# alexklwong/calibrated-backprojection-network

Measured on AMD Instinct MI355X. Metric: depth-completion frames/sec at 352x1216, higher is better.
Workload: dtype f32; 1 GPU; KITTI 352x1216, batch 32/GPU, fp32, full KBNet forward in HIP, random xavier weights; frames_per_gpu=32, global_batch=32, height=352, width=1216, n_ranks_seen=1, collective_backend=nccl, gathered_frames=32, launch=HIP graph replay, 2 concurrent sub-batch branch(es)

## Files before the change

### calibrated-backprojection-network_amd/csrc/abi.hip

```cpp
#include <stdlib.h>
#include <string.h>

#include "kbn_common.h"

namespace kbn {

KnobValue g_knobs[KNOB_COUNT];

static const char* const kKnobNames[KNOB_COUNT] = {
    "KBN_DEBUG", "KBN_FORCE_MW", "KBN_FORCE_TWB", "KBN_EPI_LDS", "KBN_NO_WINO",
    "KBN_NO_UP2X9", "KBN_NO_UP2X3", "KBN_WINO_RT",
    "KBN_NO_KB_PAIR", "KBN_NO_KB_DEPTH_FUSION", "KBN_PAIR_CAND", "KBN_S2D_DEBUG", "KBN_AUTOTUNE",
    "KBN_NO_HEAD_FUSION", "KBN_NO_SPLIT", "KBN_NO_OVERLAP", "KBN_NO_PAIR", "KBN_NO_PAIR_MID", "KBN_NO_PAIR_ENC",
    "KBN_NO_PAIR_TAIL", "KBN_NO_DEPTH_FRONT_FUSION", "KBN_FP16_ONE_TERM", "KBN_DEPTH_FRONT_FUSION", "KBN_NO_FRONT_NEXT"};

void tune_reload_env();

static void load_knobs() {
    for (int k = 0; k < KNOB_COUNT; ++k) {
        const char* v = getenv(kKnobNames[k]);
        g_knobs[k].set = (v && *v) ? 1 : 0;
        int val = 0;
        if (v && *v) {
            char* end = nullptr;
            const long parsed = strtol(v, &end, 10);
            val = (end == v) ? 1 : (int)parsed;
        }
        g_knobs[k].value = val;
    }
}

namespace {
struct KnobInit {
    KnobInit() { load_knobs(); }
} g_knob_init;
}

int device_cu_count() {
    static std::atomic<int> cache[256];
    int dev = 0;
    if (hipGetDevice(&dev) != hipSuccess) return -1;
    std::atomic<int>& slot = cache[dev & 255];
    int v = slot.load(std::memory_order_relaxed);
    if (v > 0) return v;
    if (hipDeviceGetAttribute(&v, hipDeviceAttributeMultiprocessorCount, dev) != hipSuccess || v < 1) return -1;
    slot.store(v, std::memory_order_relaxed);
    return v;
}

}

extern "C" {

int kbn_version(void) { return KBN_ABI_VERSION; }

const char* kbn_status_string(int status) {
    switch (status) {
        case KBN_OK: return "ok";
        case KBN_ERR_INVALID_ARGUMENT: return "invalid argument";
        case KBN_ERR_UNSUPPORTED: return "configuration outside the kernel limits";
        case KBN_ERR_WORKSPACE: return "buffer too small";
        case KBN_ERR_LAUNCH: return "HIP launch error";
        default: return "unknown status";
    }
}

int kbn_knob(const char* name) {
    if (!name) return 0;
    for (int k = 0; k < kbn::KNOB_COUNT; ++k)
        if (!strcmp(name, kbn::kKnobNames[k])) return kbn::g_knobs[k].value;
    return 0;
}

void kbn_reload_env(void) {
    kbn::load_knobs();
    kbn::tune_reload_env();
}

}
```

### calibrated-backprojection-network_amd/csrc/kbn_common.h

```cpp
#pragma once

#include <hip/hip_runtime.h>
#include <stdint.h>

#include <atomic>
#include <type_traits>

#include "../../include/kbnet_hip.h"

#define KBN_CHECK_LAUNCH()                                   \
    do {                                                     \
        hipError_t e__ = hipGetLastError();                  \
        if (e__ != hipSuccess) return KBN_ERR_LAUNCH;        \
    } while (0)

namespace kbn {

typedef float f32x4 __attribute__((ext_vector_type(4)));
typedef float f32x2 __attribute__((ext_vector_type(2)));

__host__ __device__ inline int ceil_div(int a, int b) { return (a + b - 1) / b; }
__host__ __device__ inline int round_up(int a, int b) { return ceil_div(a, b) * b; }

__device__ __forceinline__ float leaky_relu(float v, float slope) { return v > 0.f ? v : v * slope; }
__device__ __forceinline__ float fin_abs(float v) { const float a = fabsf(v); return a < __builtin_inff() ? a : 0.f; }

__device__ __forceinline__ unsigned wave_max_bits(float m) {
#define KBN_DPP_MAX(ctrl) m = fmaxf(m, __int_as_float(__builtin_amdgcn_update_dpp(0, __float_as_int(m), ctrl, 0xf, 0xf, true)))
    KBN_DPP_MAX(0xB1);
    KBN_DPP_MAX(0x4E);
    KBN_DPP_MAX(0x141);
    KBN_DPP_MAX(0x140);
#undef KBN_DPP_MAX
    const int v = __float_as_int(m);
    const unsigned a = (unsigned)__builtin_amdgcn_readlane(v, 0), b = (unsigned)__builtin_amdgcn_readlane(v, 16);
    const unsigned c = (unsigned)__builtin_amdgcn_readlane(v, 32), d = (unsigned)__builtin_amdgcn_readlane(v, 48);
    const unsigned ab = a > b ? a : b, cd = c > d ? c : d;
    return ab > cd ? ab : cd;
}
__device__ __forceinline__ float quad_sum(float x) {
    x += __int_as_float(__builtin_amdgcn_update_dpp(0, __float_as_int(x), 0xB1, 0xf, 0xf, true));
    x += __int_as_float(__builtin_amdgcn_update_dpp(0, __float_as_int(x), 0x4E, 0xf, 0xf, true));
    return x;
}
__device__ __forceinline__ void absmax_commit(unsigned* slot, float m) {
    const unsigned b = wave_max_bits(m);
    if ((threadIdx.x & 63) == 0) {
        if (b > __hip_atomic_load(slot, __ATOMIC_RELAXED, __HIP_MEMORY_SCOPE_AGENT)) atomicMax(slot, b);
    }
}
int absmax_frames_launch(const float* x, long long batch_stride, int n, long long per_frame, unsigned* slots, hipStream_t stream);

struct DeviceOnce {
    std::atomic<unsigned long long> done[4] = {};
};
inline int set_max_dynamic_lds(DeviceOnce& once, const void* kernel, int bytes) {
    int dev = 0;
    if (hipGetDevice(&dev) != hipSuccess) return KBN_ERR_LAUNCH;
    const unsigned long long bit = 1ull << (dev & 63);
    std::atomic<unsigned long long>& word = once.done[(dev >> 6) & 3];
    if (word.load(std::memory_order_relaxed) & bit) return KBN_OK;
    if (hipFuncSetAttribute(kernel, hipFuncAttributeMaxDynamicSharedMemorySize, bytes) != hipSuccess)
        return KBN_ERR_LAUNCH;
    word.fetch_or(bit, std::memory_order_relaxed);
    return KBN_OK;
}
template <auto K>
inline DeviceOnce lds_once;
template <auto K, int MAX_LDS, class... Args>
int launch_lds(unsigned blocks, unsigned threads, size_t lds, hipStream_t stream, const Args&... args) {
    if (int rc = set_max_dynamic_lds(lds_once<K>, reinterpret_cast<const void*>(K), MAX_LDS)) return rc;
    hipLaunchKernelGGL(K, dim3(blocks), dim3(threads), lds, stream, args...);
    return KBN_OK;
}
template <class F>
int flag_dispatch(F&& f) { return f(); }
template <class F, class... Flags>
int flag_dispatch(F&& f, bool flag, Flags... rest) {
    auto bind = [&](auto c) { return flag_dispatch([&](auto... more) { return f(c, more...); }, rest...); };
    return flag ? bind(std::true_type{}) : bind(std::false_type{});
}
int device_cu_count();

enum Knob {
    KNOB_DEBUG, KNOB_FORCE_MW, KNOB_FORCE_TWB, KNOB_EPI_LDS, KNOB_NO_WINO,
    KNOB_NO_UP2X9, KNOB_NO_UP2X3, KNOB_WINO_RT,
    KNOB_NO_KB_PAIR, KNOB_NO_KB_DEPTH_FUSION, KNOB_PAIR_CAND, KNOB_S2D_DEBUG, KNOB_AUTOTUNE,
    KNOB_NO_HEAD_FUSION, KNOB_NO_SPLIT,
    KNOB_NO_OVERLAP, KNOB_NO_PAIR, KNOB_NO_PAIR_MID, KNOB_NO_PAIR_ENC, KNOB_NO_PAIR_TAIL, KNOB_NO_DEPTH_FRONT_FUSION,
    KNOB_FP16_ONE_TERM, KNOB_DEPTH_FRONT_FUSION, KNOB_NO_FRONT_NEXT, KNOB_COUNT
};
struct KnobValue { int set, value; };
extern KnobValue g_knobs[KNOB_COUNT];
inline int knob(Knob k) { return g_knobs[k].value; }
inline bool knob_set(Knob k) { return g_knobs[k].set != 0; }

__device__ __forceinline__ int xcd_remap(int bid, int nblocks) {
    const int NX = 8;
    int xcd = bid % NX, idx = bid / NX;
    int q = nblocks / NX, r = nblocks % NX;
    int start = (xcd < r) ? xcd * (q + 1) : r * (q + 1) + (xcd - r) * q;
    return start + idx;
}

__device__ __forceinline__ int nearest_src_index(int dst, int in_size, int out_size) {
    if (in_size == out_size) return dst;
    if (out_size == 2 * in_size) return dst >> 1;
    float scale = (float)in_size / (float)out_size;
    int s = (int)floorf((float)dst * scale);
    return s < in_size - 1 ? s : in_size - 1;
}

int conv2d_launch(const kbn_conv_src* srcs, int n_src, const float* packed_weight, float* out,
                  long long out_batch_stride, int n, int out_channels, int kernel_size, int stride,
                  int in_height, int in_width, int resize, int apply_activation, float negative_slope,
                  unsigned* out_absmax, hipStream_t stream);

}
```

### calibrated-backprojection-network_amd/csrc/s2d.hip

```cpp
#include <math.h>

#include <initializer_list>

#include "kbn_common.h"
#include "s2d_pools.h"

namespace kbn {

constexpr int S2D_TW = 64, S2D_TH = 16, S2D_THREADS = 256;
constexpr int S2D_FW = S2D_TW + 2, S2D_FH = S2D_TH + 2;
constexpr int S2D_NQ = (S2D_FW + 3) / 4;
constexpr int S2D_FWP = S2D_NQ * 4;
constexpr int S2D_GS = 6;
constexpr int S2D_MAXPOOL = 8, S2D_MAXF = 8, S2D_MAXCONV = 4, S2D_MAXIN = 2, S2D_MAXR = 15;
constexpr int S2D_MAXCH = S2D_MAXF + S2D_MAXIN;
constexpr int S2D_W3 = S2D_MAXCH * 9 * 8, S2D_W1 = S2D_MAXCONV * 8 * 8;
constexpr int S2D_WFLOATS = S2D_W3 + S2D_W1;
static_assert(S2D_FH % S2D_GS == 0 && S2D_TH % 4 == 0, "tile geometry");

struct S2DParams {
    const float* x;
    long long x_bstride;
    float* out;
    float* pyramid;
    const float* wpool[S2D_MAXCONV];
    const float* wconv;
    int N, H, W, inC;
    int nmin, npool;
    int ksize[S2D_MAXPOOL];
    int nconv, nf, R, Rmin, Rmax;
    int tilesX, tilesY, nblocks;
    int dbg;
    float slope;
};

__host__ __device__ constexpr int s2d_zw(int R) { return S2D_FW + 2 * R; }
__host__ __device__ constexpr int s2d_zh(int R) { return S2D_FH + 2 * R; }
__host__ __device__ constexpr int s2d_vp(int R) { return (S2D_FWP + 2 * R + 3) / 4 * 4; }

struct DynamicPools {
    static constexpr bool is_static = false;
    static constexpr int RMAXZ = S2D_MAXR;
    __device__ static int R(const S2DParams& p) { return p.R; }
};

__device__ __forceinline__ float s2d_lrelu(float v, float slope) {
    float t = v * slope, o;
    asm("v_max_f32 %0, %1, %2" : "=v"(o) : "v"(v), "v"(t));
    return o;
}

__device__ __forceinline__ f32x4 mfma4(float a, float b, f32x4 c) {
    return __builtin_amdgcn_mfma_f32_4x4x1f32(a, b, c, 0, 0, 0);
}

template <typename CFG>
__global__ __launch_bounds__(S2D_THREADS, 2) void s2d_kernel(const S2DParams p) {
    extern __shared__ __attribute__((aligned(16))) float smem[];
    const int R = CFG::R(p);
    const int ZW = s2d_zw(R), ZH = s2d_zh(R), VP = s2d_vp(R);
    const int VPLANE = S2D_FH * VP;
    float* w3 = smem;
    float* w1 = smem + S2D_W3;
    float* zmin = smem + S2D_WFLOATS;
    float* zmax = zmin + ZH * ZW;
    float* vbuf = smem + S2D_WFLOATS + ((2 * ZH * ZW + 3) & ~3);
    float* feat = vbuf;

    const int tid = threadIdx.x, lane = tid & 63;
    const int wave = __builtin_amdgcn_readfirstlane(tid >> 6);
    const long long HW = (long long)p.H * p.W;
    const int nch = p.nf + p.inC;
    int npool = p.npool, nmin = p.nmin;
    if constexpr (CFG::is_static) { npool = CFG::NP; nmin = CFG::NMINP; }
    const float slope = p.slope;

    struct Tile { int n, oy0, ox0; };
    auto decode = [&](int t) {
        int bid = xcd_remap(t, p.nblocks);
        const int tx = bid % p.tilesX;
        bid /= p.tilesX;
        const int ty = bid % p.tilesY;
        return Tile{bid / p.tilesY, ty * S2D_TH, tx * S2D_TW};
    };
    constexpr int MAXE = (s2d_zh(CFG::RMAXZ) * s2d_zw(CFG::RMAXZ) + S2D_THREADS - 1) / S2D_THREADS;
    float vz[MAXE];
    auto z_load = [&](const Tile& tl) {
        const float* src = p.x + (long long)tl.n * p.x_bstride;
        const int Yt = tl.oy0 - 1 - R, Xl = tl.ox0 - 1 - R;
        const bool inside = Yt >= 0 && Yt + ZH <= p.H && Xl >= 0 && Xl + ZW <= p.W;
#pragma unroll
        for (int u = 0; u < MAXE; ++u) {
            const int e = u * S2D_THREADS + tid;
            const int r = e / ZW, c = e - r * ZW;
            const int Y = Yt + r, X = Xl + c;
            const bool ok = e < ZH * ZW && (inside || (Y >= 0 && Y < p.H && X >= 0 && X < p.W));
            vz[u] = ok ? src[(long long)Y * p.W + X] : -INFINITY;
        }
    };
    auto z_store = [&]() {
#pragma unroll
        for (int u = 0; u < MAXE; ++u) {
            const int e = u * S2D_THREADS + tid;
            if (e < ZH * ZW) {
                zmax[e] = vz[u];
                zmin[e] = (vz[u] == 0.f) ? 999.f : ((vz[u] == -INFINITY) ? INFINITY : vz[u]);
            }
        }
    };

    if (!p.pyramid) {
        for (int e = tid; e < S2D_W3; e += S2D_THREADS) {
            const int f = e & 7, t = (e >> 3) % 9, ch = e / 72;
            w3[e] = (f < p.nf && ch < nch) ? p.wconv[((long long)f * nch + ch) * 9 + t] : 0.f;
        }
        for (int e = tid; e < S2D_W1; e += S2D_THREADS) {
            const int f = e & 7, q = (e >> 3) & 7, i = e >> 6;
            const int cin = (i == 0) ? npool : p.nf;
            w1[e] = (i < p.nconv && f < p.nf && q < cin) ? p.wpool[i][f * cin + q] : 0.f;
        }
    }
    int tile_id = blockIdx.x;
    Tile tl = decode(tile_id);
    if (!(p.dbg & 16)) { z_load(tl); z_store(); }
    __syncthreads();

  for (;;) {
    const int n = tl.n, oy0 = tl.oy0, ox0 = tl.ox0;
    const float* xz = p.x + (long long)n * p.x_bstride;
    const bool interior = oy0 >= 1 && oy0 + S2D_TH < p.H && ox0 >= 1 && ox0 - 1 + S2D_FWP <= p.W;
    const int next_id = tile_id + (int)gridDim.x;
    const bool more = next_id < p.nblocks;

    if (p.dbg & 1) {
    } else if constexpr (CFG::is_static) {
        constexpr int NG = S2D_FH / S2D_GS;
        for (int t = tid; t < ZW * NG; t += S2D_THREADS) {
            const int g = t / ZW, c = t - g * ZW;
            auto sweep = [&](auto is_min_c, const float* zsrc) {
                constexpr bool IS_MIN = decltype(is_min_c)::value != 0;
                constexpr int RS = IS_MIN ? CFG::RMIN : CFG::RMAX;
                if constexpr (RS > 0) {
                    float m[S2D_GS + 2 * RS];
                    const float* s = zsrc + (g * S2D_GS + (CFG::RR - RS)) * ZW + c;
#pragma unroll
                    for (int i = 0; i < S2D_GS + 2 * RS; ++i) m[i] = s[i * ZW];
#pragma unroll
                    for (int j = 0; j < S2D_GS; ++j) {
                        float a = m[j + RS];
                        s2d_for<1, RS + 1>([&](auto dc) {
                            constexpr int d = decltype(dc)::value;
                            a = IS_MIN ? fminf(a, fminf(m[j + RS - d], m[j + RS + d]))
                                       : fmaxf(a, fmaxf(m[j + RS - d], m[j + RS + d]));
                            s2d_for<0, CFG::NP>([&](auto pic) {
                                constexpr int pi = decltype(pic)::value;
                                if constexpr ((pi < CFG::NMINP) == IS_MIN && CFG::radius(pi) == d)
                                    vbuf[pi * VPLANE + (g * S2D_GS + j) * VP + c] = a;
                            });
                        });
                    }
                }
            };
            sweep(IntC<1>{}, zmin);
            sweep(IntC<0>{}, zmax);
        }
    } else {
        for (int t = tid; t < ZW * S2D_FH; t += S2D_THREADS) {
            const int fr = t / ZW, c = t - fr * ZW;
            const float* smin = zmin + (fr + R) * ZW + c;
            const float* smax = zmax + (fr + R) * ZW + c;
            float a = smin[0], b = smax[0];
            for (int d = 1; d <= R; ++d) {
                if (d <= p.Rmin) a = fminf(a, fminf(smin[-d * ZW], smin[d * ZW]));
                if (d <= p.Rmax) b = fmaxf(b, fmaxf(smax[-d * ZW], smax[d * ZW]));
                for (int pi = 0; pi < npool; ++pi)
                    if ((p.ksize[pi] >> 1) == d) vbuf[pi * VPLANE + fr * VP + c] = pi < nmin ? a : b;
            }
        }
    }
    __syncthreads();
    Tile nxt = tl;
    if (more) {
        nxt = decode(next_id);
        if constexpr (CFG::is_static) {
            if (!(p.dbg & 16)) z_load(nxt);
        }
    }

    constexpr int NITEM = S2D_FH * S2D_NQ, NROUND = (NITEM + S2D_THREADS - 1) / S2D_THREADS;
    float pooled[NROUND][4][S2D_MAXPOOL];
    float xin[NROUND][S2D_MAXIN][4];
#pragma unroll
    for (int rd = 0; rd < NROUND; ++rd) {
        const int t = rd * S2D_THREADS + tid;
        const int fr = t / S2D_NQ, q = t - fr * S2D_NQ;
        const bool live = t < NITEM;
#pragma unroll
        for (int j = 0; j < 4; ++j)
#pragma unroll
            for (int pi = 0; pi < S2D_MAXPOOL; ++pi) pooled[rd][j][pi] = 0.f;
#pragma unroll
        for (int ci = 0; ci < S2D_MAXIN; ++ci)
#pragma unroll
            for (int j = 0; j < 4; ++j) {
                const int Y = oy0 - 1 + fr, X = ox0 - 1 + 4 * q + j;
                const bool inb = live && ci < p.inC && !p.pyramid && (interior || (Y >= 0 && Y < p.H && X >= 0 && X < p.W));
                xin[rd][ci][j] = inb ? xz[(long long)ci * HW + (long long)Y * p.W + X] : 0.f;
            }
        if (!live || (p.dbg & 2)) continue;
        if constexpr (CFG::is_static) {
            s2d_for<0, CFG::NP>([&](auto pic) {
                constexpr int pi = decltype(pic)::value;
                constexpr int r = CFG::radius(pi);
                constexpr bool IS_MIN = pi < CFG::NMINP;
                constexpr int OFF = CFG::RR - r;
                constexpr int A0 = OFF & ~3, SH = OFF & 3;
                constexpr int NV = 2 * r + 4, NB = (SH + NV + 3) / 4;
                static_assert(r >= 2, "the blocked window code needs pool sizes >= 5");
                f32x4 w[NB];
                const float* s = vbuf + pi * VPLANE + fr * VP + 4 * q + A0;
#pragma unroll
                for (int m = 0; m < NB; ++m) w[m] = *reinterpret_cast<const f32x4*>(s + 4 * m);
                auto v = [&](int o) { return w[(SH + o) >> 2][(SH + o) & 3]; };
                auto mn = [&](float a, float b) { return IS_MIN ? fminf(a, b) : fmaxf(a, b); };
                float core = v(3);
#pragma unroll
                for (int o = 4; o <= 2 * r; ++o) core = mn(core, v(o));
                const float l1 = mn(v(1), v(2)), l0 = mn(v(0), l1);
                const float h2 = mn(v(2 * r + 1), v(2 * r + 2)), h3 = mn(h2, v(2 * r + 3));
                float o0 = mn(core, l0), o1 = mn(core, mn(l1, v(2 * r + 1))), o2 = mn(core, mn(v(2), h2)), o3 = mn(core, h3);
                if (IS_MIN) {
                    o0 = (o0 == 999.f) ? 0.f : o0; o1 = (o1 == 999.f) ? 0.f : o1;
                    o2 = (o2 == 999.f) ? 0.f : o2; o3 = (o3 == 999.f) ? 0.f : o3;
                }
                pooled[rd][0][pi] = o0; pooled[rd][1][pi] = o1; pooled[rd][2][pi] = o2; pooled[rd][3][pi] = o3;
            });
        } else {
#pragma unroll
            for (int pi = 0; pi < S2D_MAXPOOL; ++pi) {
                if (pi >= npool) continue;
                const int r = p.ksize[pi] >> 1;
                const bool is_min = pi < nmin;
                const float* s = vbuf + pi * VPLANE + fr * VP + 4 * q + R - r;
#pragma unroll
                for (int j = 0; j < 4; ++j) {
                    float a = s[j];
                    for (int o = 1; o <= 2 * r; ++o) a = is_min ? fminf(a, s[j + o]) : fmaxf(a, s[j + o]);
                    pooled[rd][j][pi] = (is_min && a == 999.f) ? 0.f : a;
                }
            }
        }
    }
    if (p.pyramid) {
#pragma unroll
        for (int rd = 0; rd < NROUND; ++rd) {
            const int t = rd * S2D_THREADS + tid;
            const int fr = t / S2D_NQ, q = t - fr * S2D_NQ;
            if (t >= NITEM || fr < 1 || fr > S2D_TH) continue;
            const int Y = oy0 - 1 + fr;
#pragma unroll
            for (int j = 0; j < 4; ++j) {
                const int fx = 4 * q + j, X = ox0 - 1 + fx;
                if (fx < 1 || fx > S2D_TW || Y >= p.H || X >= p.W) continue;
                float* py = p.pyramid + ((long long)n * npool) * HW + (long long)Y * p.W + X;
#pragma unroll
                for (int pi = 0; pi < S2D_MAXPOOL; ++pi)
                    if (pi < npool) py[(long long)pi * HW] = pooled[rd][j][pi];
            }
        }
    }
    __syncthreads();

    if (!p.pyramid) {
#pragma unroll
        for (int rd = 0; rd < NROUND; ++rd) {
            const int t = rd * S2D_THREADS + tid;
            const int fr = t / S2D_NQ, q = t - fr * S2D_NQ;
            if (rd * S2D_THREADS + wave * 64 >= NITEM) continue;
            f32x4 h[4][2];
#pragma unroll
            for (int j = 0; j < 4; ++j) h[j][0] = h[j][1] = (f32x4){0.f, 0.f, 0.f, 0.f};
#pragma unroll
            for (int i = 0; i < S2D_MAXCONV; ++i) {
                if (i < p.nconv && !(p.dbg & 4)) {
                    float a1[8][2];
#pragma unroll
                    for (int qq = 0; qq < 8; ++qq) {
                        a1[qq][0] = w1[((i * 8 + qq) * 2 + 0) * 4 + (lane & 3)];
                        a1[qq][1] = w1[((i * 8 + qq) * 2 + 1) * 4 + (lane & 3)];
                    }
                    f32x4 g[4][2];
#pragma unroll
                    for (int j = 0; j < 4; ++j) g[j][0] = g[j][1] = (f32x4){0.f, 0.f, 0.f, 0.f};
#pragma unroll
                    for (int qq = 0; qq < 8; ++qq) {
#pragma unroll
                        for (int j = 0; j < 4; ++j) {
                            const float b = (i == 0) ? pooled[rd][j][qq] : h[j][qq >> 2][qq & 3];
                            g[j][0] = mfma4(a1[qq][0], b, g[j][0]);
                            g[j][1] = mfma4(a1[qq][1], b, g[j][1]);
                        }
                    }
#pragma unroll
                    for (int j = 0; j < 4; ++j)
#pragma unroll
                        for (int hh = 0; hh < 2; ++hh)
#pragma unroll
                            for (int f = 0; f < 4; ++f) h[j][hh][f] = s2d_lrelu(g[j][hh][f], slope);
                }
            }
            if (t < NITEM) {
                float* fo = feat + fr * S2D_FWP + 4 * q;
                if (!interior) {
                    const int Y = oy0 - 1 + fr;
                    const bool rowin = Y >= 0 && Y < p.H;
#pragma unroll
                    for (int j = 0; j < 4; ++j) {
                        const int X = ox0 - 1 + 4 * q + j;
                        if (!(rowin && X >= 0 && X < p.W)) h[j][0] = h[j][1] = (f32x4){0.f, 0.f, 0.f, 0.f};
                    }
                }
#pragma unroll
                for (int f = 0; f < S2D_MAXF; ++f)
                    if (f < p.nf)
                        *reinterpret_cast<f32x4*>(fo + f * (S2D_FH * S2D_FWP)) =
                            (f32x4){h[0][f >> 2][f & 3], h[1][f >> 2][f & 3], h[2][f >> 2][f & 3], h[3][f >> 2][f & 3]};
#pragma unroll
                for (int ci = 0; ci < S2D_MAXIN; ++ci)
                    if (ci < p.inC)
                        *reinterpret_cast<f32x4*>(fo + (p.nf + ci) * (S2D_FH * S2D_FWP)) =
                            (f32x4){xin[rd][ci][0], xin[rd][ci][1], xin[rd][ci][2], xin[rd][ci][3]};
            }
        }
    }
    __syncthreads();

    if (!p.pyramid) {
        constexpr int RW = S2D_TH / 4;
        static_assert(RW == 4, "lane mapping: 16 lanes x 4 columns per row, 4 rows per wave");
        const int lr = lane >> 4, cg = lane & 15;
        f32x4 acc[4][2];
#pragma unroll
        for (int j = 0; j < 4; ++j) acc[j][0] = acc[j][1] = (f32x4){0.f, 0.f, 0.f, 0.f};
        const float* fbase = feat + (wave * RW + lr) * S2D_FWP + 4 * cg;
        for (int ch = 0; ch < ((p.dbg & 8) ? 0 : nch); ++ch) {
            float a3[9][2], b[3][6];
            const float* wsrc = w3 + ch * 72 + (lane & 3);
#pragma unroll
            for (int tp = 0; tp < 9; ++tp) { a3[tp][0] = wsrc[tp * 8]; a3[tp][1] = wsrc[tp * 8 + 4]; }
            const float* fr = fbase + ch * (S2D_FH * S2D_FWP);
#pragma unroll
            for (int ky = 0; ky < 3; ++ky) {
                const f32x4 lo = *reinterpret_cast<const f32x4*>(fr + ky * S2D_FWP);
                const f32x2 hi = *reinterpret_cast<const f32x2*>(fr + ky * S2D_FWP + 4);
                b[ky][0] = lo[0]; b[ky][1] = lo[1]; b[ky][2] = lo[2]; b[ky][3] = lo[3]; b[ky][4] = hi[0]; b[ky][5] = hi[1];
            }
#pragma unroll
            for (int ky = 0; ky < 3; ++ky)
#pragma unroll
                for (int kx = 0; kx < 3; ++kx)
#pragma unroll
                    for (int j = 0; j < 4; ++j) {
                        acc[j][0] = mfma4(a3[ky * 3 + kx][0], b[ky][j + kx], acc[j][0]);
                        acc[j][1] = mfma4(a3[ky * 3 + kx][1], b[ky][j + kx], acc[j][1]);
                    }
        }
        const int X = ox0 + 4 * cg, Y = oy0 + wave * RW + lr;
        if (X < p.W && Y < p.H) {
            float* o = p.out + ((long long)n * p.nf) * HW + (long long)Y * p.W + X;
            const bool vec = (X + 3 < p.W) && ((p.W & 3) == 0) && ((reinterpret_cast<uintptr_t>(p.out) & 15) == 0);
#pragma unroll
            for (int f = 0; f < S2D_MAXF; ++f) {
                if (f >= p.nf) continue;
                const f32x4 v = (f32x4){s2d_lrelu(acc[0][f >> 2][f & 3], slope), s2d_lrelu(acc[1][f >> 2][f & 3], slope),
                                        s2d_lrelu(acc[2][f >> 2][f & 3], slope), s2d_lrelu(acc[3][f >> 2][f & 3], slope)};
                if (vec) {
                    *reinterpret_cast<f32x4*>(o + f * HW) = v;
                } else {
#pragma unroll
                    for (int i = 0; i < 4; ++i)
                        if (X + i < p.W) o[f * HW + i] = v[i];
                }
            }
        }
    }
    if (!more) break;
    tile_id = next_id;
    tl = nxt;
    if constexpr (!CFG::is_static) {
        if (!(p.dbg & 16)) z_load(tl);
    }
    if (!(p.dbg & 16)) z_store();
    __syncthreads();
  }
}


static int s2d_launch(S2DParams& p, const int* min_pool_sizes, int n_min, const int* max_pool_sizes,
                      int n_max, hipStream_t stream) {
    if (n_min < 0 || n_max < 0 || n_min + n_max < 1) return KBN_ERR_INVALID_ARGUMENT;
    if (n_min + n_max > S2D_MAXPOOL) return KBN_ERR_UNSUPPORTED;
    if ((n_min && !min_pool_sizes) || (n_max && !max_pool_sizes)) return KBN_ERR_INVALID_ARGUMENT;
    int R = 0;
    p.Rmin = 0; p.Rmax = 0;
    for (int i = 0; i < n_min + n_max; ++i) {
        int k = i < n_min ? min_pool_sizes[i] : max_pool_sizes[i - n_min];
        if (k < 3 || (k & 1) == 0) return KBN_ERR_INVALID_ARGUMENT;
        if (k > 2 * S2D_MAXR + 1) return KBN_ERR_UNSUPPORTED;
        p.ksize[i] = k;
        if (k / 2 > R) R = k / 2;
        if (i < n_min) { if (k / 2 > p.Rmin) p.Rmin = k / 2; } else { if (k / 2 > p.Rmax) p.Rmax = k / 2; }
    }
    for (int i = n_min + n_max; i < S2D_MAXPOOL; ++i) p.ksize[i] = 1;
    p.nmin = n_min;
    p.npool = n_min + n_max;
    p.R = R;
    p.tilesX = ceil_div(p.W, S2D_TW);
    p.tilesY = ceil_div(p.H, S2D_TH);
    const size_t z_floats = ((size_t)2 * s2d_zh(R) * s2d_zw(R) + 3) & ~(size_t)3;
    const size_t v_floats = (size_t)p.npool * S2D_FH * s2d_vp(R);
    const size_t feat_floats = (size_t)S2D_MAXCH * S2D_FH * S2D_FWP;
    const size_t lds = sizeof(float) * (S2D_WFLOATS + z_floats + (v_floats > feat_floats ? v_floats : feat_floats));
    if (lds > 160 * 1024) return KBN_ERR_UNSUPPORTED;
    const long long blocks = (long long)p.tilesX * p.tilesY * p.N;
    if (blocks > 0x7fffffffLL) return KBN_ERR_UNSUPPORTED;
    p.nblocks = (int)blocks;
    p.dbg = knob(KNOB_S2D_DEBUG);
    auto matches = [&](int nm, std::initializer_list<int> ks) {
        if (p.nmin != nm || p.npool != (int)ks.size()) return false;
        int i = 0;
        for (int k : ks)
            if (p.ksize[i++] != k) return false;
        return true;
    };
    int cus = device_cu_count();
    if (cus < 1) cus = 256;
    const long long per_cu = (2 * lds <= 160 * 1024) ? 2 : 1;
    const unsigned grid = (unsigned)(blocks < per_cu * cus ? blocks : per_cu * cus);
    int rc;
    if (matches(5, {5, 7, 9, 11, 13, 15, 17})) rc = launch_lds<s2d_kernel<KittiPools>, 160 * 1024>(grid, S2D_THREADS, lds, stream, p);
    else if (matches(2, {15, 17, 23, 27, 29})) rc = launch_lds<s2d_kernel<VoidPools>, 160 * 1024>(grid, S2D_THREADS, lds, stream, p);
    else if (matches(3, {15, 17, 19, 23, 27})) rc = launch_lds<s2d_kernel<VoidTrainPools>, 160 * 1024>(grid, S2D_THREADS, lds, stream, p);
    else rc = launch_lds<s2d_kernel<DynamicPools>, 160 * 1024>(grid, S2D_THREADS, lds, stream, p);
    if (rc != KBN_OK) return rc;
    KBN_CHECK_LAUNCH();
    return KBN_OK;
}

}

extern "C" {

int kbn_s2d_forward(const float* x, const float* const* w_pool_convs, const float* w_conv, float* out,
                    int n, int height, int width, int input_channels, const int* min_pool_sizes,
                    int n_min, const int* max_pool_sizes, int n_max, int n_convolution, int n_filter,
                    float negative_slope, kbn_stream_t stream) {
    using namespace kbn;
    if (!x || !w_pool_convs || !w_conv || !out) return KBN_ERR_INVALID_ARGUMENT;
    if (n < 1 || height < 1 || width < 1 || input_channels < 1 || n_convolution < 1 || n_filter < 1)
        return KBN_ERR_INVALID_ARGUMENT;
    if (n_filter > S2D_MAXF || input_channels > S2D_MAXIN || n_convolution > S2D_MAXCONV)
        return KBN_ERR_UNSUPPORTED;
    if (!(negative_slope >= 0.f && negative_slope <= 1.f)) return KBN_ERR_UNSUPPORTED;
    S2DParams p{};
    p.x = x;
    p.x_bstride = (long long)input_channels * height * width;
    p.out = out;
    p.pyramid = nullptr;
    for (int i = 0; i < S2D_MAXCONV; ++i) {
        p.wpool[i] = i < n_convolution ? w_pool_convs[i] : w_pool_convs[0];
        if (i < n_convolution && !w_pool_convs[i]) return KBN_ERR_INVALID_ARGUMENT;
    }
    p.wconv = w_conv;
    p.N = n; p.H = height; p.W = width; p.inC = input_channels;
    p.nconv = n_convolution; p.nf = n_filter; p.slope = negative_slope;
    return s2d_launch(p, min_pool_sizes, n_min, max_pool_sizes, n_max, (hipStream_t)stream);
}

int kbn_s2d_pyramid(const float* x_depth, long long batch_stride, float* pyramid, int n, int height,
                    int width, const int* min_pool_sizes, int n_min, const int* max_pool_sizes, int n_max,
                    kbn_stream_t stream) {
    using namespace kbn;
    if (!x_depth || !pyramid || n < 1 || height < 1 || width < 1) return KBN_ERR_INVALID_ARGUMENT;
    S2DParams p{};
    p.x = x_depth;
    p.x_bstride = batch_stride;
    p.out = nullptr;
    p.pyramid = pyramid;
    p.N = n; p.H = height; p.W = width; p.inC = 1;
    p.nconv = 1; p.nf = 1; p.slope = 0.f;
    return s2d_launch(p, min_pool_sizes, n_min, max_pool_sizes, n_max, (hipStream_t)stream);
}

}
```

Baseline: 2954 frames/s.

## Run sparse-to-dense kernel with 8 waves per block for static pool configs

Adds a 512-thread variant of the sparse-to-dense (S2D) kernel, used by default for static, non-pyramid pool configurations. The 1x1 and 3x3 convolution stages are remapped so each lane handles 2 pixels instead of 4, the min/max pool sweep group shrinks, and the 3x3 weights are re-laid out in LDS so each lane loads them as contiguous pairs. The goal is more waves in flight per CU and lower per-thread register pressure, to hide LDS and MFMA latency in this front-end stage. The cost is more redundant weight loads per pixel and smaller vector stores. A new KBN_S2D_NARROW knob restores the old path.

```diff
diff --git a/calibrated-backprojection-network_amd/csrc/abi.hip b/calibrated-backprojection-network_amd/csrc/abi.hip
--- a/calibrated-backprojection-network_amd/csrc/abi.hip
+++ b/calibrated-backprojection-network_amd/csrc/abi.hip
@@ -12,7 +12,8 @@
     "KBN_NO_UP2X9", "KBN_NO_UP2X3", "KBN_WINO_RT",
     "KBN_NO_KB_PAIR", "KBN_NO_KB_DEPTH_FUSION", "KBN_PAIR_CAND", "KBN_S2D_DEBUG", "KBN_AUTOTUNE",
     "KBN_NO_HEAD_FUSION", "KBN_NO_SPLIT", "KBN_NO_OVERLAP", "KBN_NO_PAIR", "KBN_NO_PAIR_MID", "KBN_NO_PAIR_ENC",
-    "KBN_NO_PAIR_TAIL", "KBN_NO_DEPTH_FRONT_FUSION", "KBN_FP16_ONE_TERM", "KBN_DEPTH_FRONT_FUSION", "KBN_NO_FRONT_NEXT"};
+    "KBN_NO_PAIR_TAIL", "KBN_NO_DEPTH_FRONT_FUSION", "KBN_FP16_ONE_TERM", "KBN_DEPTH_FRONT_FUSION", "KBN_NO_FRONT_NEXT",
+    "KBN_S2D_NARROW"};
 
 void tune_reload_env();
 
diff --git a/calibrated-backprojection-network_amd/csrc/kbn_common.h b/calibrated-backprojection-network_amd/csrc/kbn_common.h
--- a/calibrated-backprojection-network_amd/csrc/kbn_common.h
+++ b/calibrated-backprojection-network_amd/csrc/kbn_common.h
@@ -88,7 +88,7 @@
     KNOB_NO_KB_PAIR, KNOB_NO_KB_DEPTH_FUSION, KNOB_PAIR_CAND, KNOB_S2D_DEBUG, KNOB_AUTOTUNE,
     KNOB_NO_HEAD_FUSION, KNOB_NO_SPLIT,
     KNOB_NO_OVERLAP, KNOB_NO_PAIR, KNOB_NO_PAIR_MID, KNOB_NO_PAIR_ENC, KNOB_NO_PAIR_TAIL, KNOB_NO_DEPTH_FRONT_FUSION,
-    KNOB_FP16_ONE_TERM, KNOB_DEPTH_FRONT_FUSION, KNOB_NO_FRONT_NEXT, KNOB_COUNT
+    KNOB_FP16_ONE_TERM, KNOB_DEPTH_FRONT_FUSION, KNOB_NO_FRONT_NEXT, KNOB_S2D_NARROW, KNOB_COUNT
 };
 struct KnobValue { int set, value; };
 extern KnobValue g_knobs[KNOB_COUNT];
diff --git a/calibrated-backprojection-network_amd/csrc/s2d.hip b/calibrated-backprojection-network_amd/csrc/s2d.hip
--- a/calibrated-backprojection-network_amd/csrc/s2d.hip
+++ b/calibrated-backprojection-network_amd/csrc/s2d.hip
@@ -7,16 +7,17 @@
 
 namespace kbn {
 
-constexpr int S2D_TW = 64, S2D_TH = 16, S2D_THREADS = 256;
+constexpr int S2D_TW = 64, S2D_TH = 16;
+constexpr int S2D_THREADS = 256, S2D_THREADS_WIDE = 512;
 constexpr int S2D_FW = S2D_TW + 2, S2D_FH = S2D_TH + 2;
 constexpr int S2D_NQ = (S2D_FW + 3) / 4;
 constexpr int S2D_FWP = S2D_NQ * 4;
-constexpr int S2D_GS = 6;
+__host__ __device__ constexpr int s2d_gs(int threads) { return threads > 256 ? 3 : 6; }
 constexpr int S2D_MAXPOOL = 8, S2D_MAXF = 8, S2D_MAXCONV = 4, S2D_MAXIN = 2, S2D_MAXR = 15;
 constexpr int S2D_MAXCH = S2D_MAXF + S2D_MAXIN;
 constexpr int S2D_W3 = S2D_MAXCH * 9 * 8, S2D_W1 = S2D_MAXCONV * 8 * 8;
 constexpr int S2D_WFLOATS = S2D_W3 + S2D_W1;
-static_assert(S2D_FH % S2D_GS == 0 && S2D_TH % 4 == 0, "tile geometry");
+static_assert(S2D_FH % s2d_gs(S2D_THREADS) == 0 && S2D_FH % s2d_gs(S2D_THREADS_WIDE) == 0 && S2D_TH % 8 == 0, "tile geometry");
 
 struct S2DParams {
     const float* x;
@@ -54,8 +55,11 @@
     return __builtin_amdgcn_mfma_f32_4x4x1f32(a, b, c, 0, 0, 0);
 }
 
-template <typename CFG>
-__global__ __launch_bounds__(S2D_THREADS, 2) void s2d_kernel(const S2DParams p) {
+template <typename CFG, int THREADS>
+__global__ __launch_bounds__(THREADS, THREADS / 128) void s2d_kernel(const S2DParams p) {
+    static_assert(THREADS == S2D_THREADS || THREADS == S2D_THREADS_WIDE, "4 or 8 waves");
+    constexpr int GS = s2d_gs(THREADS);
+    constexpr bool W3_BY_LANE = THREADS > S2D_THREADS;
     extern __shared__ __attribute__((aligned(16))) float smem[];
     const int R = CFG::R(p);
     const int ZW = s2d_zw(R), ZH = s2d_zh(R), VP = s2d_vp(R);
@@ -83,15 +87,17 @@
         const int ty = bid % p.tilesY;
         return Tile{bid / p.tilesY, ty * S2D_TH, tx * S2D_TW};
     };
-    constexpr int MAXE = (s2d_zh(CFG::RMAXZ) * s2d_zw(CFG::RMAXZ) + S2D_THREADS - 1) / S2D_THREADS;
+    constexpr int MAXE = (s2d_zh(CFG::RMAXZ) * s2d_zw(CFG::RMAXZ) + THREADS - 1) / THREADS;
     float vz[MAXE];
     auto z_load = [&](const Tile& tl) {
         const float* src = p.x + (long long)tl.n * p.x_bstride;
         const int Yt = tl.oy0 - 1 - R, Xl = tl.ox0 - 1 - R;
         const bool inside = Yt >= 0 && Yt + ZH <= p.H && Xl >= 0 && Xl + ZW <= p.W;
+        int zt = tid;
+        if constexpr (THREADS > S2D_THREADS) asm volatile("" : "+v"(zt));
 #pragma unroll
         for (int u = 0; u < MAXE; ++u) {
-            const int e = u * S2D_THREADS + tid;
+            const int e = u * THREADS + zt;
             const int r = e / ZW, c = e - r * ZW;
             const int Y = Yt + r, X = Xl + c;
             const bool ok = e < ZH * ZW && (inside || (Y >= 0 && Y < p.H && X >= 0 && X < p.W));
@@ -101,7 +107,7 @@
     auto z_store = [&]() {
 #pragma unroll
         for (int u = 0; u < MAXE; ++u) {
-            const int e = u * S2D_THREADS + tid;
+            const int e = u * THREADS + tid;
             if (e < ZH * ZW) {
                 zmax[e] = vz[u];
                 zmin[e] = (vz[u] == 0.f) ? 999.f : ((vz[u] == -INFINITY) ? INFINITY : vz[u]);
@@ -110,11 +116,12 @@
     };
 
     if (!p.pyramid) {
-        for (int e = tid; e < S2D_W3; e += S2D_THREADS) {
+        for (int e = tid; e < S2D_W3; e += THREADS) {
             const int f = e & 7, t = (e >> 3) % 9, ch = e / 72;
-            w3[e] = (f < p.nf && ch < nch) ? p.wconv[((long long)f * nch + ch) * 9 + t] : 0.f;
-        }
-        for (int e = tid; e < S2D_W1; e += S2D_THREADS) {
+            const int slot = W3_BY_LANE ? ch * 72 + (f & 3) * 18 + t * 2 + (f >> 2) : e;
+            w3[slot] = (f < p.nf && ch < nch) ? p.wconv[((long long)f * nch + ch) * 9 + t] : 0.f;
+        }
+        for (int e = tid; e < S2D_W1; e += THREADS) {
             const int f = e & 7, q = (e >> 3) & 7, i = e >> 6;
             const int cin = (i == 0) ? npool : p.nf;
             w1[e] = (i < p.nconv && f < p.nf && q < cin) ? p.wpool[i][f * cin + q] : 0.f;
@@ -134,19 +141,19 @@
 
     if (p.dbg & 1) {
     } else if constexpr (CFG::is_static) {
-        constexpr int NG = S2D_FH / S2D_GS;
-        for (int t = tid; t < ZW * NG; t += S2D_THREADS) {
+        constexpr int NG = S2D_FH / GS;
+        for (int t = tid; t < ZW * NG; t += THREADS) {
             const int g = t / ZW, c = t - g * ZW;
             auto sweep = [&](auto is_min_c, const float* zsrc) {
                 constexpr bool IS_MIN = decltype(is_min_c)::value != 0;
                 constexpr int RS = IS_MIN ? CFG::RMIN : CFG::RMAX;
                 if constexpr (RS > 0) {
-                    float m[S2D_GS + 2 * RS];
-                    const float* s = zsrc + (g * S2D_GS + (CFG::RR - RS)) * ZW + c;
-#pragma unroll
-                    for (int i = 0; i < S2D_GS + 2 * RS; ++i) m[i] = s[i * ZW];
-#pragma unroll
-                    for (int j = 0; j < S2D_GS; ++j) {
+                    float m[GS + 2 * RS];
+                    const float* s = zsrc + (g * GS + (CFG::RR - RS)) * ZW + c;
+#pragma unroll
+                    for (int i = 0; i < GS + 2 * RS; ++i) m[i] = s[i * ZW];
+#pragma unroll
+                    for (int j = 0; j < GS; ++j) {
                         float a = m[j + RS];
                         s2d_for<1, RS + 1>([&](auto dc) {
                             constexpr int d = decltype(dc)::value;
@@ -155,7 +162,7 @@
                             s2d_for<0, CFG::NP>([&](auto pic) {
                                 constexpr int pi = decltype(pic)::value;
                                 if constexpr ((pi < CFG::NMINP) == IS_MIN && CFG::radius(pi) == d)
-                                    vbuf[pi * VPLANE + (g * S2D_GS + j) * VP + c] = a;
+                                    vbuf[pi * VPLANE + (g * GS + j) * VP + c] = a;
                             });
                         });
                     }
@@ -165,7 +172,7 @@
             sweep(IntC<0>{}, zmax);
         }
     } else {
-        for (int t = tid; t < ZW * S2D_FH; t += S2D_THREADS) {
+        for (int t = tid; t < ZW * S2D_FH; t += THREADS) {
             const int fr = t / ZW, c = t - fr * ZW;
             const float* smin = zmin + (fr + R) * ZW + c;
             const float* smax = zmax + (fr + R) * ZW + c;
@@ -187,12 +194,12 @@
         }
     }
 
-    constexpr int NITEM = S2D_FH * S2D_NQ, NROUND = (NITEM + S2D_THREADS - 1) / S2D_THREADS;
+    constexpr int NITEM = S2D_FH * S2D_NQ, NROUND = (NITEM + THREADS - 1) / THREADS;
     float pooled[NROUND][4][S2D_MAXPOOL];
     float xin[NROUND][S2D_MAXIN][4];
 #pragma unroll
     for (int rd = 0; rd < NROUND; ++rd) {
-        const int t = rd * S2D_THREADS + tid;
+        const int t = rd * THREADS + tid;
         const int fr = t / S2D_NQ, q = t - fr * S2D_NQ;
         const bool live = t < NITEM;
 #pragma unroll
@@ -254,7 +261,7 @@
     if (p.pyramid) {
 #pragma unroll
         for (int rd = 0; rd < NROUND; ++rd) {
-            const int t = rd * S2D_THREADS + tid;
+            const int t = rd * THREADS + tid;
             const int fr = t / S2D_NQ, q = t - fr * S2D_NQ;
             if (t >= NITEM || fr < 1 || fr > S2D_TH) continue;
             const int Y = oy0 - 1 + fr;
@@ -272,59 +279,70 @@
     __syncthreads();
 
     if (!p.pyramid) {
+        constexpr int PJ = THREADS > S2D_THREADS ? 2 : 4;
 #pragma unroll
         for (int rd = 0; rd < NROUND; ++rd) {
-            const int t = rd * S2D_THREADS + tid;
+            const int t = rd * THREADS + tid;
             const int fr = t / S2D_NQ, q = t - fr * S2D_NQ;
-            if (rd * S2D_THREADS + wave * 64 >= NITEM) continue;
-            f32x4 h[4][2];
-#pragma unroll
-            for (int j = 0; j < 4; ++j) h[j][0] = h[j][1] = (f32x4){0.f, 0.f, 0.f, 0.f};
-#pragma unroll
-            for (int i = 0; i < S2D_MAXCONV; ++i) {
-                if (i < p.nconv && !(p.dbg & 4)) {
-                    float a1[8][2];
-#pragma unroll
-                    for (int qq = 0; qq < 8; ++qq) {
-                        a1[qq][0] = w1[((i * 8 + qq) * 2 + 0) * 4 + (lane & 3)];
-                        a1[qq][1] = w1[((i * 8 + qq) * 2 + 1) * 4 + (lane & 3)];
+            if (rd * THREADS + wave * 64 >= NITEM) continue;
+            const bool item = t < NITEM;
+            float* fo = feat + fr * S2D_FWP + 4 * q;
+#pragma unroll
+            for (int j0 = 0; j0 < 4; j0 += PJ) {
+                f32x4 h[PJ][2];
+#pragma unroll
+                for (int j = 0; j < PJ; ++j) h[j][0] = h[j][1] = (f32x4){0.f, 0.f, 0.f, 0.f};
+#pragma unroll
+                for (int i = 0; i < S2D_MAXCONV; ++i) {
+                    if (i < p.nconv && !(p.dbg & 4)) {
+                        float a1[8][2];
+#pragma unroll
+                        for (int qq = 0; qq < 8; ++qq) {
+                            a1[qq][0] = w1[((i * 8 + qq) * 2 + 0) * 4 + (lane & 3)];
+                            a1[qq][1] = w1[((i * 8 + qq) * 2 + 1) * 4 + (lane & 3)];
+                        }
+                        f32x4 g[PJ][2];
+#pragma unroll
+                        for (int j = 0; j < PJ; ++j) g[j][0] = g[j][1] = (f32x4){0.f, 0.f, 0.f, 0.f};
+#pragma unroll
+                        for (int qq = 0; qq < 8; ++qq) {
+#pragma unroll
+                            for (int j = 0; j < PJ; ++j) {
+                                const float b = (i == 0) ? pooled[rd][j0 + j][qq] : h[j][qq >> 2][qq & 3];
+                                g[j][0] = mfma4(a1[qq][0], b, g[j][0]);
+                                g[j][1] = mfma4(a1[qq][1], b, g[j][1]);
+                            }
+                        }
+#pragma unroll
+                        for (int j = 0; j < PJ; ++j)
+#pragma unroll
+                            for (int hh = 0; hh < 2; ++hh)
+#pragma unroll
+                                for (int f = 0; f < 4; ++f) h[j][hh][f] = s2d_lrelu(g[j][hh][f], slope);
                     }
-                    f32x4 g[4][2];
-#pragma unroll
-                    for (int j = 0; j < 4; ++j) g[j][0] = g[j][1] = (f32x4){0.f, 0.f, 0.f, 0.f};
-#pragma unroll
-                    for (int qq = 0; qq < 8; ++qq) {
-#pragma unroll
-                        for (int j = 0; j < 4; ++j) {
-                            const float b = (i == 0) ? pooled[rd][j][qq] : h[j][qq >> 2][qq & 3];
-                            g[j][0] = mfma4(a1[qq][0], b, g[j][0]);
-                            g[j][1] = mfma4(a1[qq][1], b, g[j][1]);
+                }
+                if (item) {
+                    if (!interior) {
+                        const int Y = oy0 - 1 + fr;
+                        const bool rowin = Y >= 0 && Y < p.H;
+#pragma unroll
+                        for (int j = 0; j < PJ; ++j) {
+                            const int X = ox0 - 1 + 4 * q + j0 + j;
+                            if (!(rowin && X >= 0 && X < p.W)) h[j][0] = h[j][1] = (f32x4){0.f, 0.f, 0.f, 0.f};
                         }
                     }
 #pragma unroll
-                    for (int j = 0; j < 4; ++j)
-#pragma unroll
-                        for (int hh = 0; hh < 2; ++hh)
-#pragma unroll
-                            for (int f = 0; f < 4; ++f) h[j][hh][f] = s2d_lrelu(g[j][hh][f], slope);
-                }
-            }
-            if (t < NITEM) {
-                float* fo = feat + fr * S2D_FWP + 4 * q;
-                if (!interior) {
-                    const int Y = oy0 - 1 + fr;
-                    const bool rowin = Y >= 0 && Y < p.H;
-#pragma unroll
-                    for (int j = 0; j < 4; ++j) {
-                        const int X = ox0 - 1 + 4 * q + j;
-                        if (!(rowin && X >= 0 && X < p.W)) h[j][0] = h[j][1] = (f32x4){0.f, 0.f, 0.f, 0.f};
-                    }
-                }
-#pragma unroll
-                for (int f = 0; f < S2D_MAXF; ++f)
-                    if (f < p.nf)
-                        *reinterpret_cast<f32x4*>(fo + f * (S2D_FH * S2D_FWP)) =
-                            (f32x4){h[0][f >> 2][f & 3], h[1][f >> 2][f & 3], h[2][f >> 2][f & 3], h[3][f >> 2][f & 3]};
+                    for (int f = 0; f < S2D_MAXF; ++f)
+                        if (f < p.nf) {
+                            float* d = fo + f * (S2D_FH * S2D_FWP) + j0;
+                            if constexpr (PJ == 4)
+                                *reinterpret_cast<f32x4*>(d) = (f32x4){h[0][f >> 2][f & 3], h[1][f >> 2][f & 3], h[2][f >> 2][f & 3], h[3][f >> 2][f & 3]};
+                            else
+                                *reinterpret_cast<f32x2*>(d) = (f32x2){h[0][f >> 2][f & 3], h[1][f >> 2][f & 3]};
+                        }
+                }
+            }
+            if (item) {
 #pragma unroll
                 for (int ci = 0; ci < S2D_MAXIN; ++ci)
                     if (ci < p.inC)
@@ -336,49 +354,67 @@
     __syncthreads();
 
     if (!p.pyramid) {
-        constexpr int RW = S2D_TH / 4;
-        static_assert(RW == 4, "lane mapping: 16 lanes x 4 columns per row, 4 rows per wave");
-        const int lr = lane >> 4, cg = lane & 15;
-        f32x4 acc[4][2];
-#pragma unroll
-        for (int j = 0; j < 4; ++j) acc[j][0] = acc[j][1] = (f32x4){0.f, 0.f, 0.f, 0.f};
-        const float* fbase = feat + (wave * RW + lr) * S2D_FWP + 4 * cg;
+        constexpr int RW = S2D_TH / (THREADS / 64);
+        constexpr int LPR = 64 / RW, PX = S2D_TW / LPR;
+        static_assert((RW == 4 && PX == 4) || (RW == 2 && PX == 2), "lane mapping: LPR lanes x PX columns per row, RW rows per wave");
+        const int lr = lane / LPR, cg = lane % LPR;
+        f32x4 acc[PX][2];
+#pragma unroll
+        for (int j = 0; j < PX; ++j) acc[j][0] = acc[j][1] = (f32x4){0.f, 0.f, 0.f, 0.f};
+        const float* fbase = feat + (wave * RW + lr) * S2D_FWP + PX * cg;
         for (int ch = 0; ch < ((p.dbg & 8) ? 0 : nch); ++ch) {
-            float a3[9][2], b[3][6];
-            const float* wsrc = w3 + ch * 72 + (lane & 3);
-#pragma unroll
-            for (int tp = 0; tp < 9; ++tp) { a3[tp][0] = wsrc[tp * 8]; a3[tp][1] = wsrc[tp * 8 + 4]; }
+            float a3[9][2], b[3][PX + 2];
+            if constexpr (W3_BY_LANE) {
+                const float* wsrc = w3 + ch * 72 + (lane & 3) * 18;
+#pragma unroll
+                for (int tp = 0; tp < 9; ++tp) {
+                    const f32x2 a = *reinterpret_cast<const f32x2*>(wsrc + tp * 2);
+                    a3[tp][0] = a[0]; a3[tp][1] = a[1];
+                }
+            } else {
+                const float* wsrc = w3 + ch * 72 + (lane & 3);
+#pragma unroll
+                for (int tp = 0; tp < 9; ++tp) { a3[tp][0] = wsrc[tp * 8]; a3[tp][1] = wsrc[tp * 8 + 4]; }
+            }
             const float* fr = fbase + ch * (S2D_FH * S2D_FWP);
 #pragma unroll
             for (int ky = 0; ky < 3; ++ky) {
-                const f32x4 lo = *reinterpret_cast<const f32x4*>(fr + ky * S2D_FWP);
-                const f32x2 hi = *reinterpret_cast<const f32x2*>(fr + ky * S2D_FWP + 4);
-                b[ky][0] = lo[0]; b[ky][1] = lo[1]; b[ky][2] = lo[2]; b[ky][3] = lo[3]; b[ky][4] = hi[0]; b[ky][5] = hi[1];
+                if constexpr (PX == 4) {
+                    const f32x4 lo = *reinterpret_cast<const f32x4*>(fr + ky * S2D_FWP);
+                    const f32x2 hi = *reinterpret_cast<const f32x2*>(fr + ky * S2D_FWP + 4);
+                    b[ky][0] = lo[0]; b[ky][1] = lo[1]; b[ky][2] = lo[2]; b[ky][3] = lo[3]; b[ky][4] = hi[0]; b[ky][5] = hi[1];
+                } else {
+                    const f32x2 lo = *reinterpret_cast<const f32x2*>(fr + ky * S2D_FWP);
+                    const f32x2 hi = *reinterpret_cast<const f32x2*>(fr + ky * S2D_FWP + 2);
+                    b[ky][0] = lo[0]; b[ky][1] = lo[1]; b[ky][2] = hi[0]; b[ky][3] = hi[1];
+                }
             }
 #pragma unroll
             for (int ky = 0; ky < 3; ++ky)
 #pragma unroll
                 for (int kx = 0; kx < 3; ++kx)
 #pragma unroll
-                    for (int j = 0; j < 4; ++j) {
+                    for (int j = 0; j < PX; ++j) {
                         acc[j][0] = mfma4(a3[ky * 3 + kx][0], b[ky][j + kx], acc[j][0]);
                         acc[j][1] = mfma4(a3[ky * 3 + kx][1], b[ky][j + kx], acc[j][1]);
                     }
         }
-        const int X = ox0 + 4 * cg, Y = oy0 + wave * RW + lr;
+        const int X = ox0 + PX * cg, Y = oy0 + wave * RW + lr;
         if (X < p.W && Y < p.H) {
             float* o = p.out + ((long long)n * p.nf) * HW + (long long)Y * p.W + X;
-            const bool vec = (X + 3 < p.W) && ((p.W & 3) == 0) && ((reinterpret_cast<uintptr_t>(p.out) & 15) == 0);
+            const bool vec = (X + PX - 1 < p.W) && ((p.W & (PX - 1)) == 0) && ((reinterpret_cast<uintptr_t>(p.out) & (4 * PX - 1)) == 0);
 #pragma unroll
             for (int f = 0; f < S2D_MAXF; ++f) {
                 if (f >= p.nf) continue;
-                const f32x4 v = (f32x4){s2d_lrelu(acc[0][f >> 2][f & 3], slope), s2d_lrelu(acc[1][f >> 2][f & 3], slope),
-                                        s2d_lrelu(acc[2][f >> 2][f & 3], slope), s2d_lrelu(acc[3][f >> 2][f & 3], slope)};
+                float v[PX];
+#pragma unroll
+                for (int i = 0; i < PX; ++i) v[i] = s2d_lrelu(acc[i][f >> 2][f & 3], slope);
                 if (vec) {
-                    *reinterpret_cast<f32x4*>(o + f * HW) = v;
+                    if constexpr (PX == 4) *reinterpret_cast<f32x4*>(o + f * HW) = (f32x4){v[0], v[1], v[2], v[3]};
+                    else *reinterpret_cast<f32x2*>(o + f * HW) = (f32x2){v[0], v[1]};
                 } else {
 #pragma unroll
-                    for (int i = 0; i < 4; ++i)
+                    for (int i = 0; i < PX; ++i)
                         if (X + i < p.W) o[f * HW + i] = v[i];
                 }
             }
@@ -437,11 +473,18 @@
     if (cus < 1) cus = 256;
     const long long per_cu = (2 * lds <= 160 * 1024) ? 2 : 1;
     const unsigned grid = (unsigned)(blocks < per_cu * cus ? blocks : per_cu * cus);
+    const bool wide = !p.pyramid && !knob(KNOB_S2D_NARROW);
+    auto launch = [&](auto cfg) {
+        using CFG = decltype(cfg);
+        if constexpr (CFG::is_static)
+            if (wide) return launch_lds<s2d_kernel<CFG, S2D_THREADS_WIDE>, 160 * 1024>(grid, S2D_THREADS_WIDE, lds, stream, p);
+        return launch_lds<s2d_kernel<CFG, S2D_THREADS>, 160 * 1024>(grid, S2D_THREADS, lds, stream, p);
+    };
     int rc;
-    if (matches(5, {5, 7, 9, 11, 13, 15, 17})) rc = launch_lds<s2d_kernel<KittiPools>, 160 * 1024>(grid, S2D_THREADS, lds, stream, p);
-    else if (matches(2, {15, 17, 23, 27, 29})) rc = launch_lds<s2d_kernel<VoidPools>, 160 * 1024>(grid, S2D_THREADS, lds, stream, p);
-    else if (matches(3, {15, 17, 19, 23, 27})) rc = launch_lds<s2d_kernel<VoidTrainPools>, 160 * 1024>(grid, S2D_THREADS, lds, stream, p);
-    else rc = launch_lds<s2d_kernel<DynamicPools>, 160 * 1024>(grid, S2D_THREADS, lds, stream, p);
+    if (matches(5, {5, 7, 9, 11, 13, 15, 17})) rc = launch(KittiPools{});
+    else if (matches(2, {15, 17, 23, 27, 29})) rc = launch(VoidPools{});
+    else if (matches(3, {15, 17, 19, 23, 27})) rc = launch(VoidTrainPools{});
+    else rc = launch(DynamicPools{});
     if (rc != KBN_OK) return rc;
     KBN_CHECK_LAUNCH();
     return KBN_OK;
```

New measurement: 2984 frames/s, median of 6. 1.01x the previous value.
